# ahmetaa/fast-dnn

Measured on AMD Instinct MI355X. Metric: acoustic frames/sec (whole node), 7x2048->8000 nnet, higher is better.
Workload: dtype int8 (u8 activations x s8 weights -> int32; fp32 layer 0 and soft-max)

## Files before the change

### fast-dnn_amd/api.py

```python
from __future__ import annotations

import ctypes as C
import os
import subprocess
from typing import Optional, Sequence

import numpy as np

_HERE = os.path.dirname(os.path.abspath(__file__))
LIB_PATH = os.environ.get("FDNN_LIB") or os.path.join(_HERE, "lib", "libfast-dnn.so")
CSRC = os.path.join(_HERE, "csrc")

FDNN_OK, FDNN_E_ARG, FDNN_E_IO, FDNN_E_FORMAT, FDNN_E_DEVICE, FDNN_E_NOMEM, FDNN_E_STATE = 0, -1, -2, -3, -4, -5, -6


class FdnnError(RuntimeError):
    def __init__(self, code: int, msg: str):
        super().__init__(f"fdnn error {code}: {msg}")
        self.code = code


def build(verbose: bool = False) -> str:
    jobs = str(max(1, min(8, os.cpu_count() or 1)))
    subprocess.check_call(["make", "-C", CSRC, "-j", jobs, "all"] + ([] if verbose else ["-s"]))
# ... 15 lines not shown
    "fdnn_model_load_on": (C.c_int, [C.c_char_p, C.c_float, C.c_int, C.POINTER(C.c_void_p)]),
    "fdnn_model_free": (None, [C.c_void_p]),
    "fdnn_model_input_dim": (C.c_int, [C.c_void_p]),
    "fdnn_model_output_dim": (C.c_int, [C.c_void_p]),
    "fdnn_model_hidden_dim": (C.c_int, [C.c_void_p]),
    "fdnn_model_layer_count": (C.c_int, [C.c_void_p]),
    "fdnn_model_layer_dim": (C.c_int, [C.c_void_p, C.c_int]),
    "fdnn_model_device": (C.c_int, [C.c_void_p]),
    "fdnn_model_set_l0_fma": (C.c_int, [C.c_void_p, C.c_int]),
    "fdnn_debug_set_l0_kernel": (C.c_int, [C.c_void_p, C.c_int]),
    "fdnn_debug_set_chain": (C.c_int, [C.c_int, C.c_int]),
    "fdnn_model_chain_faults": (C.c_int, [C.c_void_p, C.POINTER(C.c_ulonglong)]),
    "fdnn_debug_set_pp": (C.c_int, [C.c_int, C.c_int]),
    "fdnn_debug_set_ppo": (C.c_int, [C.c_int]),
    "fdnn_debug_launch_name_count": (C.c_int, []),
    "fdnn_debug_launch_name": (C.c_char_p, [C.c_int, C.POINTER(C.c_int)]),
    "fdnn_debug_launch_record": (C.c_int, [C.c_int]),
    "fdnn_debug_launch_reset": (C.c_int, []),
    "fdnn_debug_launch_counts": (C.c_int, [C.POINTER(C.c_ulonglong), C.c_int]),
    "fdnn_debug_raise_fuse_fault": (C.c_int, [C.c_void_p, C.c_int]),
    "fdnn_device_shared": (C.c_int, [C.c_int]),
    "fdnn_debug_set_fuse": (C.c_int, [C.c_int]),
    "fdnn_debug_set_l0_list_cap": (C.c_int, [C.c_void_p, C.c_int]),
    "fdnn_debug_chain_clocks": (C.c_int, [C.c_void_p, C.POINTER(C.c_longlong), C.c_int]),
    "fdnn_calculate": (C.c_int, [C.c_void_p, _c_f32p, C.c_int, C.c_int, C.c_int, _c_f32p]),
    "fdnn_calculate_device": (C.c_int, [C.c_void_p, C.c_void_p, C.c_int, C.c_void_p, C.c_void_p]),
    "fdnn_calculate_lazy": (C.c_int, [C.c_void_p, _c_f32p, C.c_int, C.c_int, _c_i8p, _c_f32p]),
    "fdnn_calculate_lazy_bits": (C.c_int, [C.c_void_p, _c_f32p, C.c_int, C.c_int, C.POINTER(C.c_uint64), _c_f32p]),
    "fdnn_calculate_lazy_bits_device": (C.c_int, [C.c_void_p, C.c_void_p, C.c_int, C.c_void_p, C.c_void_p, C.c_void_p]),
    "fdnn_ctx_create": (C.c_int, [C.c_void_p, C.c_int, C.c_int, C.POINTER(C.c_void_p)]),
    "fdnn_ctx_free": (None, [C.c_void_p]),
    "fdnn_ctx_frame_count": (C.c_int, [C.c_void_p]),
    "fdnn_ctx_output_dim": (C.c_int, [C.c_void_p]),
    "fdnn_ctx_forward_hidden": (C.c_int, [C.c_void_p, _c_f32p]),
    "fdnn_ctx_forward_hidden_device": (C.c_int, [C.c_void_p, C.c_void_p, C.c_void_p]),
    "fdnn_ctx_lazy_output": (C.c_int, [C.c_void_p, C.c_int, _c_i8p, _c_f32p]),
    "fdnn_ctx_lazy_output_batch": (C.c_int, [C.c_void_p, C.c_int, C.c_int, _c_i8p, _c_f32p]),
    "fdnn_ctx_lazy_output_batch_device": (C.c_int, [C.c_void_p, C.c_int, C.c_int, C.c_void_p, C.c_void_p, C.c_void_p]),
    "fdnn_ctx_output": (C.c_int, [C.c_void_p, _c_f32p]),
    "fdnn_ctx_output_device": (C.c_int, [C.c_void_p, C.c_void_p, C.c_void_p]),
    "fdnn_ctx_read_hidden": (C.c_int, [C.c_void_p, _c_u8p]),
    "fdnn_server_create": (C.c_int, [C.c_void_p, C.c_int, C.c_int, C.POINTER(C.c_void_p)]),
    "fdnn_server_free": (None, [C.c_void_p]),
    "fdnn_server_set_linger_us": (C.c_int, [C.c_void_p, C.c_int]),
    "fdnn_server_submit_device": (C.c_int, [C.c_void_p, C.c_void_p, C.c_int, C.c_void_p, C.c_void_p, C.POINTER(C.c_uint64)]),
    "fdnn_server_submit": (C.c_int, [C.c_void_p, _c_f32p, C.c_int, _c_i8p, _c_f32p, C.POINTER(C.c_uint64)]),
# ... 119 lines not shown
def device_shared(device: int = 0) -> bool:
    r = int(lib().fdnn_device_shared(int(device)))
    if r < 0:
        _check(r)
    return r == 1


def set_fuse(mode: int) -> None:
    _check(lib().fdnn_debug_set_fuse(int(mode)))


def set_chain(mode: int, min_frames: int = 0) -> None:
    _check(lib().fdnn_debug_set_chain(int(mode), int(min_frames)))


def set_pp(mode: int, min_frames: int = 0) -> None:
    _check(lib().fdnn_debug_set_pp(int(mode), int(min_frames)))


def set_ppo(mode: int) -> None:
    _check(lib().fdnn_debug_set_ppo(int(mode)))


LAUNCH_ABLATION, LAUNCH_LOAD_TIME = 1, 2


def launch_names() -> dict:
    L = lib()
    out = {}
    for i in range(L.fdnn_debug_launch_name_count()):
        flags = C.c_int(0)
        name = L.fdnn_debug_launch_name(i, C.byref(flags)).decode()
        out[name] = flags.value
    return out


def launch_record(on: bool = True) -> None:
    _check(lib().fdnn_debug_launch_record(1 if on else 0))


def launch_reset() -> None:
    _check(lib().fdnn_debug_launch_reset())


def launch_counts(nonzero: bool = True) -> dict:
    L = lib()
# ... 601 lines not shown
```

### fast-dnn_amd/csrc/fdnn_debug.cpp

```cpp
#include <hip/hip_runtime.h>

#include <algorithm>
#include <atomic>
#include <cstring>
#include <mutex>
#include <string>
#include <vector>

#include "fdnn_internal.hpp"

using namespace fdnn;

struct fdnn_host_model {
  fdnn::HostModel hm;
};

namespace fdnn {
const LaunchNameInfo kLaunchNames[kLaunchNameCount] = {
#define FDNN_X(id, name, flags) {name, flags},
    FDNN_LAUNCH_NAMES(FDNN_X)
#undef FDNN_X
#define FDNN_G(out, shape, branch, name, abl) {name, abl},
        FDNN_GEMM_LAUNCH_NAMES(FDNN_G)
#undef FDNN_G
// ... 32 lines not shown
int fdnn_debug_lazy_expand(float *out, const float *comp, int count, int O, int stride, const uint64_t *bits, int mode) {
  if (!out || !comp || !bits || count < 0 || O <= 0 || stride <= 0 || stride > O + 1 || mode < 0 || mode > 2) return fail(FDNN_E_ARG, "bad argument");
  lazy_expand_force_scalar(mode == 1);
  if (mode == 2) {
    if (stride > O) return fail(FDNN_E_ARG, "the in-place form needs stride <= O");
    std::memmove(out + size_t(count) * size_t(O) - size_t(count) * size_t(stride), comp, sizeof(float) * size_t(count) * size_t(stride));
    fdnn::lazy_expand_rows(out, count, size_t(O), size_t(stride), bits);
  } else {
    fdnn::lazy_expand_rows_from(out, comp, count, size_t(O), size_t(stride), bits);
  }
  lazy_expand_force_scalar(false);
  return FDNN_OK;
}

int fdnn_debug_set_l0_list_cap(fdnn_model *m, int cap) {
  if (!m || cap < 0) return fail(FDNN_E_ARG, "bad argument");
  std::lock_guard<std::mutex> lk(m->mu);
  for (fdnn_ctx *c : m->pool) destroy_ctx(c);
  m->pool.clear();
  m->l0_list_cap = cap;
  return FDNN_OK;
}

int fdnn_debug_set_pp(int mode, int min_frames) {
  if (mode < -1 || mode > 1) return fail(FDNN_E_ARG, "pp mode must be -1, 0 or 1");
  fdnn::qpp_set_mode(mode, min_frames);
  return FDNN_OK;
}

int fdnn_debug_raise_fuse_fault(fdnn_model *m, int value) {
  if (!m) return fail(FDNN_E_ARG, "null model");
  if (!m->h_fuse_fault) return fail(FDNN_E_STATE, "this model has no fault word");
  __atomic_store_n(m->h_fuse_fault, value ? 1ull : 0ull, __ATOMIC_RELAXED);
  if (!value) m->fuse_fault_said = false;
  return FDNN_OK;
}

int fdnn_debug_set_ppo(int mode) {
  if (mode < -1 || mode > 1) return fail(FDNN_E_ARG, "ppo mode must be -1, 0 or 1");
  fdnn::qppo_set_mode(mode);
  return FDNN_OK;
}

int fdnn_debug_launch_name_count(void) { return fdnn::kLaunchNameCount; }

const char *fdnn_debug_launch_name(int index, int *flags) {
// ... 352 lines not shown
```

### fast-dnn_amd/csrc/fdnn_kernels.hpp

```cpp
#pragma once
#include <hip/hip_runtime.h>

#include <cstdint>
#include <vector>

#include "fdnn_note.hpp"

#ifdef FDNN_ABLATION
#include <cstdlib>
#define FDNN_TUNE_ENV(name) std::getenv(name)
#else
#define FDNN_TUNE_ENV(name) static_cast<const char *>(nullptr)
#if (defined(FDNN_GEMM_DEBUG) && FDNN_GEMM_DEBUG) || (defined(FDNN_L0S_DEBUG) && FDNN_L0S_DEBUG) || (defined(FDNN_L0_DEBUG) && FDNN_L0_DEBUG) || \
    (defined(FDNN_CHAIN_CLK) && FDNN_CHAIN_CLK) || defined(FDNN_L0S_CLK) || defined(FDNN_GEMM_PAD)
#error "ablation / clock builds need -DFDNN_ABLATION (tools/build_variant.sh)"
#endif
#endif

namespace fdnn {

constexpr int kMaxFrameTile = 320;
constexpr int kPartialNodes = 64;

struct L0Params {
// ... 15 lines not shown
  float *park;
  int j_pad, jc;
  int n_ld, h_ld;
  const float *wnorm;
  uint32_t *scr_count;
  uint16_t *scr_list;
  unsigned long long *scr_stats;
  int8_t *xd;
  float *xstat;
  const int8_t *wd;
  const float *wstat;
  uint2 *glist;
  uint32_t *glist_count;
  int glist_cap;
  const uint32_t *luthalf;
  float *dbg_t;
  float *dbg_dd;
};
constexpr int kL0ScreenCap = 4096;
void launch_l0(const L0Params &p, hipStream_t s);
bool l0_split_ok(int D, int H);
size_t l0_split_plane_bytes(int D, int rows_ld);
void launch_l0_split(const L0Params &p, hipStream_t s);
void l0_split_build_weights(const float *w, const float *wnorm, const uint8_t *lut2, int H, int D, int h_ld, std::vector<int8_t> *planes,
                            std::vector<float> *stat, std::vector<uint32_t> *half);
int l0_chunk_rows(int D);
int l0_chain_node_tile();
void launch_l0_weight_image(const float *w, float *wt, int H, int D, int j_pad, int h_ld, hipStream_t s);

int qgemm_frame_tile(int rows_pad, int n);
int qgemm_node_tile(int rows_pad, int n, bool output);
int qgemm_debug_flags();

struct QGemmParams {
  const int8_t *w;
  const int8_t *a;
  const float *bias;
  const int32_t *wsum;
  const int32_t *fix_grp;
  const void *fix_ent;
  const uint8_t *lut;
  const uint8_t *lut2;
  int rows, rows_pad, K, n, n_pad;
  int ldw, lda;
  int frame_tile;
  int small;
// ... 91 lines not shown
```

### fast-dnn_amd/csrc/fdnn_l0s.hip

```cpp
#include <atomic>
#include <cmath>
#include <cstdlib>
#include <limits>
#include <type_traits>
#include <vector>

#include "fdnn_device.hpp"
#include "fdnn_kernels.hpp"

namespace fdnn {

namespace {

#ifndef FDNN_L0S_DEBUG
#define FDNN_L0S_DEBUG 0
#endif
constexpr float kU = 5.9604645e-8f;
constexpr int kSplitW = 32;

[[maybe_unused]] __device__ __forceinline__ bool split_tile_of_block(int node_tiles, int frame_tiles, int &bx, int &by) {
  const int b = blockIdx.x, xcd = b & 7, slot = b >> 3;
  bx = slot % node_tiles;
  by = xcd + 8 * (slot / node_tiles);
  return by < frame_tiles;
}

constexpr int kDigFrames = 8;
__global__ __launch_bounds__(256) void l0_digits_kernel(L0Params p, int KC, int J, int JP) {
  extern __shared__ __attribute__((aligned(16))) float dig_smem[];
  const int D = p.D, ld = D + 1;
  float *xs = dig_smem;
  float *cf_s = dig_smem + kDigFrames * ld;
  const int tid = threadIdx.x, f0 = blockIdx.x * kDigFrames;
  if (blockIdx.x == 0 && tid < 2) p.glist_count[tid] = 0u;
  const int quads = D >> 2;
  {
    float4 raw[4], sh[4], sc[4];
    int rowq[4];
#pragma unroll
    for (int it = 0; it < 4; ++it) {
      const int i = tid + it * 256;
      const int row = i / quads, q = i - row * quads, f = f0 + row;
      const bool in = i < kDigFrames * quads;
      rowq[it] = in ? row * ld + 4 * q : -1;
      raw[it] = make_float4(0.f, 0.f, 0.f, 0.f);
      sh[it] = raw[it];
      sc[it] = raw[it];
      if (in && f < p.n) {
// ... 75 lines not shown
      d1[e4] = w1; d2[e4] = w2; d3[e4] = w3;
    }
    const int f = f0 + row;
    if (f >= p.n_ld) continue;
    const size_t blocks = static_cast<size_t>(p.n_ld >> 5);
#pragma unroll
    for (int pl = 0; pl < 3; ++pl) {
      const uint32_t *d = pl == 0 ? d1 : pl == 1 ? d2 : d3;
      char *base = reinterpret_cast<char *>(p.xd) + ((static_cast<size_t>(kc) * 3 + pl) * blocks + (f >> 5)) * 1024 + hh * 512 + (f & 31) * 16;
      *reinterpret_cast<uint4 *>(base) = make_uint4(d[0], d[1], d[2], d[3]);
    }
  }
}

constexpr int kSTF = 128, kSStages = 3;
template <int WN>
struct SplitCfg {
  static constexpr int TN = 64 * WN, NW = 4 * WN, THREADS = 64 * NW;
  static constexpr int PIECES = 12 + 6 * WN;
  static constexpr int STAGE = PIECES * 1024;
  static constexpr int RING = STAGE * kSStages;
  static constexpr int HALF_OFF = RING;
  static constexpr int STAT_OFF = RING + 11 * 1024;
  static constexpr int LDS = STAT_OFF + 3 * 1024;
  static constexpr int TS = TN + 16;
  static constexpr int PPW = (PIECES + NW - 1) / NW;
  static_assert(kSTF * TS + 16 + 2 * kL0ScreenCap <= RING, "epilogue tile and flag list must fit in the dead ring");
};
static_assert(4 * kLut2Size <= 11 * 1024, "half-step table area");

template <int WN, bool DBG = false>
__global__ __launch_bounds__(256 * WN, 3 - WN) void l0_split_kernel(L0Params p, int KC, int CPC) {
#if defined(__HIP_DEVICE_COMPILE__)
  using Cfg = SplitCfg<WN>;
  constexpr int kSTN = Cfg::TN, kSStage = Cfg::STAGE, kSTS = Cfg::TS, kSHalfOff = Cfg::HALF_OFF, kSStatOff = Cfg::STAT_OFF, NW = Cfg::NW;
  extern __shared__ __attribute__((aligned(16))) char smem[];
  const int tid = threadIdx.x, lane = tid & 63;
  const int wave = __builtin_amdgcn_readfirstlane(tid >> 6);
  const int l32 = lane & 31, h = lane >> 5;
  const int wf = wave & 3, wn = wave >> 2;
  const int node_tiles = p.h_ld / kSTN, frame_tiles = (p.n_rows + kSTF - 1) / kSTF;
  int bx, by;
  if (!split_tile_of_block(node_tiles, frame_tiles, bx, by)) return;
  const int f0 = by * kSTF, n0 = bx * kSTN;
  const int xblocks = p.n_ld >> 5, wblocks = p.h_ld >> 5;
#ifdef FDNN_L0S_CLK
  long long tc[12];
  tc[0] = __builtin_readcyclecounter();
#define L0S_TS(i) tc[i] = __builtin_readcyclecounter()
#else
#define L0S_TS(i)
#endif

  {
    const __amdgpu_buffer_rsrc_t rsrc_half =
        __builtin_amdgcn_make_buffer_rsrc(const_cast<uint32_t *>(p.luthalf), 0, (4 * kLut2Size + 15) & ~15, 0x00020000);
#pragma unroll
    for (int i = 0; i < 14; ++i) {
      if (i % NW != wave) continue;
      if (i < 11) {
        __builtin_amdgcn_raw_ptr_buffer_load_lds(rsrc_half, FDNN_LDS_PTR(smem + kSHalfOff + i * 1024), 16, lane * 16, i * 1024, 0, 0);
      } else {
        const int q = i - 11;
        const __amdgpu_buffer_rsrc_t rsrc_st =
            __builtin_amdgcn_make_buffer_rsrc(const_cast<float *>(p.xstat + static_cast<size_t>(q) * p.n_ld + f0), 0, kSTF * 4, 0x00020000);
        __builtin_amdgcn_raw_ptr_buffer_load_lds(rsrc_st, FDNN_LDS_PTR(smem + kSStatOff + q * 1024), 16, lane * 16, 0, 0, 0);
      }
    }
  }
  const __amdgpu_buffer_rsrc_t rsrc_x =
      __builtin_amdgcn_make_buffer_rsrc(const_cast<int8_t *>(p.xd), 0, static_cast<unsigned>(KC) * 3u * static_cast<unsigned>(xblocks) * 1024u, 0x00020000);
  const __amdgpu_buffer_rsrc_t rsrc_w = __builtin_amdgcn_make_buffer_rsrc(
      const_cast<int8_t *>(p.wd), 0, static_cast<unsigned>(KC) * 3u * static_cast<unsigned>(wblocks) * 1024u, 0x00020000);
  const int voff = lane * 16;
  const int my_pieces = (Cfg::PIECES - wave + NW - 1) / NW;
  auto stage_piece = [&](int kc, int buf, int t) {
    char *base = smem + buf * kSStage;
    const int i = wave + NW * t;
    if (i >= Cfg::PIECES) return;
    if (i < 12) {
      const int pl = i >> 2, q = i & 3;
      __builtin_amdgcn_raw_ptr_buffer_load_lds(rsrc_x, FDNN_LDS_PTR(base + i * 1024), 16, voff, ((kc * 3 + pl) * xblocks + (f0 >> 5) + q) * 1024, 0, 0);
    } else {
      const int j = i - 12, pl = j / (2 * WN), q = j % (2 * WN);
      __builtin_amdgcn_raw_ptr_buffer_load_lds(rsrc_w, FDNN_LDS_PTR(base + i * 1024), 16, voff, ((kc * 3 + pl) * wblocks + (n0 >> 5) + q) * 1024, 0, 0);
    }
  };
  auto stage = [&](int kc, int buf) {
#pragma unroll
    for (int t = 0; t < Cfg::PPW; ++t) stage_piece(kc, buf, t);
  };
  auto wait_stages = [&](int stages) {
    if (stages == 0) {
      asm volatile("s_waitcnt vmcnt(0) lgkmcnt(0)" ::: "memory");
    } else if (Cfg::PIECES % NW == 0) {
      if (stages == 1)
        asm volatile("s_waitcnt vmcnt(%0) lgkmcnt(0)" ::"n"(Cfg::PPW) : "memory");
      else
        asm volatile("s_waitcnt vmcnt(%0) lgkmcnt(0)" ::"n"(2 * Cfg::PPW) : "memory");
    } else if (my_pieces == Cfg::PPW) {
// ... 12 lines not shown
  stage(1, 1);
  stage(2, 2);
  asm volatile("" ::: "memory");

  constexpr int kP0Off = 0x40000000;
  v16i P0[2], P1[2], P2[2];
  uint32_t A[2][16];
#pragma unroll
  for (int s = 0; s < 2; ++s)
#pragma unroll
    for (int r = 0; r < 16; ++r) {
      P0[s][r] = kP0Off; P1[s][r] = 0; P2[s][r] = 0;
      A[s][r] = 0u;
    }
  auto chain_end = [&](int s) {
#pragma unroll
    for (int r = 0; r < 16; ++r) {
      P1[s][r] += P0[s][r] << 8;
      P0[s][r] = kP0Off;
    }
  };
  v4i xa[2][3], wb[2][3][2];
  auto load_plane = [&](int buf, int set, int pl) {
    const char *sb = smem + buf * kSStage;
    xa[set][pl] = *reinterpret_cast<const v4i *>(sb + (pl * 4 + wf) * 1024 + lane * 16);
#pragma unroll
    for (int s = 0; s < 2; ++s) wb[set][pl][s] = *reinterpret_cast<const v4i *>(sb + 12288 + (pl * 2 * WN + wn * 2 + s) * 1024 + lane * 16);
  };
  auto load_frags = [&](int buf, int set) {
#pragma unroll
    for (int pl = 0; pl < 3; ++pl) load_plane(buf, set, pl);
  };
  auto sample_part = [&](int ss, int r0, int r1, bool on) {
    if ((FDNN_L0S_DEBUG & 1) || !on) return;
#pragma unroll
    for (int r = r0; r < r1; ++r) asm volatile("v_sad_u32 %0, %1, 2.0, %0" : "+v"(A[ss][r]) : "v"(P0[ss][r]));
  };
#define FDNN_L0S_FENCE __builtin_amdgcn_sched_barrier(0)
  auto mfma_group = [&](int set, int s, int ss, bool on, auto x0, auto x1, auto x2, auto x3, auto x4) {
    FDNN_L0S_FENCE;
    P0[s] = __builtin_amdgcn_mfma_i32_32x32x32_i8(xa[set][0], wb[set][0][s], P0[s], 0, 0, 0);
    if (FDNN_L0S_DEBUG & 2) {
      sample_part(ss, 0, 16, on);
      x0(); x1(); x2(); x3(); x4();
      return;
    }
    FDNN_L0S_FENCE;
// ... 15 lines not shown
    sample_part(ss, 9, 12, on);
    x3();
    FDNN_L0S_FENCE;
    P2[s] = __builtin_amdgcn_mfma_i32_32x32x32_i8(xa[set][1], wb[set][1][s], P2[s], 0, 0, 0);
    FDNN_L0S_FENCE;
    sample_part(ss, 12, 16, on);
    x4();
    FDNN_L0S_FENCE;
    P2[s] = __builtin_amdgcn_mfma_i32_32x32x32_i8(xa[set][2], wb[set][0][s], P2[s], 0, 0, 0);
    FDNN_L0S_FENCE;
  };
  auto nothing = [] {};

  wait_stages(2);
  __builtin_amdgcn_s_barrier();
  asm volatile("" ::: "memory");
  load_frags(0, 0);
  L0S_TS(1);
  auto chunk = [&](int kc, auto set_c, auto first_c, bool chain_start) {
    constexpr int set = decltype(set_c)::value;
    constexpr bool first = decltype(first_c)::value;
    if (chain_start) chain_end(0);
    mfma_group(set, 0, 1, !first, nothing, nothing, nothing, nothing, nothing);
    const bool more = kc + 1 < KC, refill = kc + 3 < KC && !(FDNN_L0S_DEBUG & 8);
    if (more) {
      wait_stages(kc + 2 < KC ? 1 : 0);
      if (!(FDNN_L0S_DEBUG & 16)) __builtin_amdgcn_s_barrier();
      asm volatile("" ::: "memory");
    }
    if (chain_start) chain_end(1);
    const int nb = (kc + 1) % 3;
    mfma_group(
        set, 1, 0, true, [&] { if (more && !(FDNN_L0S_DEBUG & 32)) load_plane(nb, set ^ 1, 0); if (refill) stage_piece(kc + 3, kc % 3, 0); },
        [&] { if (more && !(FDNN_L0S_DEBUG & 32)) load_plane(nb, set ^ 1, 1); if (refill) stage_piece(kc + 3, kc % 3, 1); },
        [&] { if (more && !(FDNN_L0S_DEBUG & 32)) load_plane(nb, set ^ 1, 2); if (refill) stage_piece(kc + 3, kc % 3, 2); },
        [&] { if (refill && Cfg::PPW > 3) stage_piece(kc + 3, kc % 3, 3); }, [&] { if (refill && Cfg::PPW > 4) stage_piece(kc + 3, kc % 3, 4); });
  };
  using C0 = std::integral_constant<int, 0>;
  using C1 = std::integral_constant<int, 1>;
  chunk(0, C0{}, std::true_type{}, false);
  chunk(1, C1{}, std::false_type{}, false);
  for (int kc = 2, in_chain = 2; kc < KC; kc += 2, in_chain += 2) {
    const bool chain_start = in_chain == CPC;
    if (chain_start) in_chain = 0;
    chunk(kc, C0{}, std::false_type{}, chain_start);
    chunk(kc + 1, C1{}, std::false_type{}, false);
  }
  sample_part(1, 0, 16, true);
  chain_end(0);
  chain_end(1);
  L0S_TS(2);

  __syncthreads();
  const char *half_b = smem + kSHalfOff + 4 * kLut2Half;
  const float *rf_s = reinterpret_cast<const float *>(smem + kSStatOff);
  const float *xn_s = rf_s + 256, *af_s = rf_s + 512;
  uint8_t *tile = reinterpret_cast<uint8_t *>(smem);
  uint32_t *scr_n = reinterpret_cast<uint32_t *>(tile + kSTF * kSTS);
  uint16_t *scr_l = reinterpret_cast<uint16_t *>(tile + kSTF * kSTS + 16);
  if (tid == 0) *scr_n = 0;
  const float fD = static_cast<float>(p.D);
  const float c2 = 1.001f * (0.5f * fD * fD + 2.0f * fD) * kU;
  const float kA = 1.00001f * 256.0f * 1.002f * kU * (kSplitW + 3);
  const float kS = 100.001f * 1.002f * kU * (kSplitW / 2 + 2 + c2);
  float bias100[2], rn100[2], kSw2[2], bn2[2], eb2[2];
  bool node_in[2];
#pragma unroll
  for (int s = 0; s < 2; ++s) {
    const int node = n0 + wn * 64 + s * 32 + l32;
    node_in[s] = node < p.H;
    const float b = node_in[s] ? p.bias[node] : 0.0f;
    bias100[s] = 100.0f * b;
    rn100[s] = 100.0f * (node_in[s] ? p.wstat[node] : 0.0f);
    kSw2[s] = kS * (node_in[s] ? p.wstat[p.h_ld + node] : 0.0f);
    bn2[s] = 1.00001f * (node_in[s] ? p.wstat[2 * p.h_ld + node] : 0.0f);
    eb2[s] = 100.001f * 10.0f * kU * fabsf(b);
  }
  uint32_t valid = 0;
#pragma unroll
  for (int r = 0; r < 16; ++r) {
    const bool row_in = f0 + wf * 32 + 8 * (r >> 2) + 4 * h + (r & 3) < p.n;
    valid |= (row_in && node_in[0] ? 1u : 0u) << r;
    valid |= (row_in && node_in[1] ? 1u : 0u) << (16 + r);
  }
  float tt[2][16], sg[2][16];
  uint32_t ent[2][16];
#pragma unroll
  for (int r = 0; r < 16; ++r) {
    const float rf = rf_s[wf * 32 + 8 * (r >> 2) + 4 * h + (r & 3)];
#pragma unroll
    for (int s = 0; s < 2; ++s) {
      const float v = fmaf(static_cast<float>(P2[s][r]), 0.00390625f, static_cast<float>(P1[s][r]));
      sg[s][r] = rf * rn100[s];
      tt[s][r] = fmaf(v, sg[s][r], bias100[s]);
      const int u = max(-kLut2Half, min(kLut2Half, static_cast<int>(tt[s][r] + tt[s][r])));
      ent[s][r] = *reinterpret_cast<const uint32_t *>(half_b + 4 * u);
    }
  }
  uint32_t scr_mask = 0;
#pragma unroll
  for (int r = 0; r < 16; ++r) {
    const int row = wf * 32 + 8 * (r >> 2) + 4 * h + (r & 3);
    const float xn = xn_s[row], af = af_s[row];
#pragma unroll
    for (int s = 0; s < 2; ++s) {
      const float t = tt[s][r], sig = sg[s][r];
      tile[row * kSTS + wn * 64 + s * 32 + l32] = static_cast<uint8_t>(ent[s][r]);
      if (!(FDNN_L0S_DEBUG & 4)) {
        const float e = __builtin_amdgcn_fractf(t) - 0.5f;
        const float Dd = fmaf(fabsf(t), 12.0f * kU, fmaf(sig, fmaf(kA, static_cast<float>(A[s][r]), af + bn2[s]), fmaf(kSw2[s], xn, eb2[s]))) + 1e-30f;
        const float gate = __builtin_bit_cast(float, ent[s][r] & 0xffff0000u);
        const float m = fmaxf(fmaxf(fabsf(e), gate), fabsf(t) - 641.0f);
        const bool flag = !(m > Dd) | !(fabsf(t) < 1.0e9f);
        scr_mask |= flag ? (1u << (16 * s + r)) : 0u;
        if (DBG && ((valid >> (16 * s + r)) & 1u)) {
          const size_t o = static_cast<size_t>(f0 + row) * p.H + (n0 + wn * 64 + s * 32 + l32);
          p.dbg_t[o] = t;
          p.dbg_dd[o] = Dd;
        }
      }
    }
  }
  scr_mask &= valid;
  L0S_TS(3);
  __syncthreads();
  L0S_TS(4);
  {
    const int mine = __popc(scr_mask);
    int incl = mine;
#pragma unroll
    for (int off = 1; off < 64; off <<= 1) {
      const int v = __shfl_up(incl, off);
      if (lane >= off) incl += v;
    }
    const int wave_total = __shfl(incl, 63);
    if (wave_total) {
      uint32_t base = 0;
      if (lane == 63) base = atomicAdd(scr_n, static_cast<uint32_t>(wave_total));
      base = __shfl(base, 63);
      uint32_t at = base + static_cast<uint32_t>(incl - mine);
      uint32_t m = scr_mask;
      while (m) {
        const int i = __ffs(m) - 1;
        m &= m - 1;
        const int r = i & 15, sb2 = i >> 4;
        const int row = wf * 32 + 8 * (r >> 2) + 4 * h + (r & 3), col = wn * 64 + sb2 * 32 + l32;
        if (at < static_cast<uint32_t>(kL0ScreenCap)) scr_l[at] = static_cast<uint16_t>(row * kSTN + col);
        ++at;
      }
    }
  }
#pragma unroll
  for (int q = 0; q < kSTF * (kSTN / 16) / Cfg::THREADS; ++q) {
    const int item = tid + q * Cfg::THREADS, row = item / (kSTN / 16), c16 = (item % (kSTN / 16)) * 16;
    const int f = f0 + row;
    if (f < p.n_rows && n0 + c16 < p.H)
      *reinterpret_cast<uint4 *>(p.act_out + static_cast<size_t>(f) * p.act_ld + n0 + c16) = *reinterpret_cast<const uint4 *>(tile + row * kSTS + c16);
  }
  __syncthreads();
  {
    const uint32_t cnt = *scr_n;
    uint32_t *gbase_s = scr_n + 1;
    if (tid == 0) {
      uint32_t gb = 0xffffffffu, fill_from = 0xffffffffu;
      if (cnt != 0 && cnt <= static_cast<uint32_t>(kL0ScreenCap)) {
        gb = atomicAdd(p.glist_count, cnt);
        if (gb + cnt > static_cast<uint32_t>(p.glist_cap)) {
          fill_from = gb;
          gb = 0xffffffffu;
        }
      }
      if (cnt != 0 && gb == 0xffffffffu) {
        p.scr_count[by * (p.h_ld / 128) + (n0 >> 7)] = cnt;
        atomicAdd(p.glist_count + 1, 1u);
      }
      *gbase_s = gb;
      gbase_s[1] = fill_from;
    }
    __syncthreads();
    const uint32_t gb = *gbase_s, fill_from = gbase_s[1];
    if (fill_from < static_cast<uint32_t>(p.glist_cap))
      for (uint32_t i = fill_from + tid; i < static_cast<uint32_t>(p.glist_cap); i += Cfg::THREADS) p.glist[i] = make_uint2(0xffffffffu, 0xffffffffu);
    if (gb != 0xffffffffu)
      for (uint32_t i = tid; i < cnt; i += Cfg::THREADS) {
        const uint32_t e = scr_l[i];
        p.glist[gb + i] = make_uint2(static_cast<uint32_t>(f0) + e / kSTN, static_cast<uint32_t>(n0) + e % kSTN);
      }
  }
#ifdef FDNN_L0S_CLK
  L0S_TS(5);
  if (p.scr_stats && lane == 0 && wave == 0 && (blockIdx.x == 0 || blockIdx.x == gridDim.x / 2 + 3)) {
    unsigned long long *o = p.scr_stats + 4 + (blockIdx.x == 0 ? 0 : 12);
    for (int i = 0; i < 6; ++i) o[i] = static_cast<unsigned long long>(tc[i] - tc[0]);
  }
#endif
#endif
}

}

bool l0_split_ok(int D, int H) { return D >= 64 && D <= 496 && (D & 3) == 0 && (H & 15) == 0; }
int l0_split_chain_pad(int D) { return (D / 4 + 63) / 64 * 64; }
int l0_split_chunks(int D) { return 4 * l0_split_chain_pad(D) / 32; }
size_t l0_split_plane_bytes(int D, int rows_ld) { return static_cast<size_t>(l0_split_chunks(D)) * 3 * static_cast<size_t>(rows_ld / 32) * 1024; }
size_t l0_split_half_bytes() { return (4 * size_t(kLut2Size) + 15) & ~size_t(15); }

void l0_split_build_weights(const float *w, const float *wnorm, const uint8_t *lut2, int H, int D, int h_ld, std::vector<int8_t> *planes,
                            std::vector<float> *stat, std::vector<uint32_t> *half) {
  const int J = D / 4, JP = l0_split_chain_pad(D);
  planes->assign(l0_split_plane_bytes(D, h_ld), 0);
  stat->assign(static_cast<size_t>(3) * h_ld, 0.0f);
  half->assign(l0_split_half_bytes() / 4, 0);
  auto at = [&](int u) { return lut2[std::max(-kLut2Half, std::min(kLut2Half, u)) + kLut2Half]; };
  for (int u = -kLut2Half; u <= kLut2Half; ++u) {
    const int mag = u < 0 ? -u : u;
    bool same;
// ... 22 lines not shown
      const int c = pp / JP, j = pp - c * JP, k = 4 * j + c;
      if (j >= J) continue;
      const long W = degenerate ? 0 : std::lrint(static_cast<double>(row[k]) * static_cast<double>(cn));
      n1W += static_cast<double>(W < 0 ? -W : W);
      const int x3 = static_cast<int8_t>(W & 0xff), r = static_cast<int>((W - x3) >> 8), x2 = static_cast<int8_t>(r & 0xff), x1 = (r - x2) >> 8;
      n1W2 += std::abs(x2);
      n1W3 += std::abs(x3);
      const int digit[3] = {x1, x2, x3};
      const int kc = pp >> 5, hh = (pp >> 4) & 1, e = pp & 15;
      for (int pl = 0; pl < 3; ++pl)
        (*planes)[((static_cast<size_t>(kc) * 3 + pl) * blocks + (n >> 5)) * 1024 + hh * 512 + (n & 31) * 16 + e] = static_cast<int8_t>(digit[pl]);
    }
    const double b_n = (u * (kSplitW + 3) * m * 0.502 * n1W / 65536.0 + std::ldexp(0.5 * n1W, -32) + std::ldexp(128.0 * (n1W2 + n1W3), -24) +
                        std::ldexp(128.0 * n1W3, -32)) * 1.002;
    auto up = [](double v) {
      float f = static_cast<float>(v);
      if (static_cast<double>(f) < v) f = std::nextafter(f, std::numeric_limits<float>::infinity());
      return f;
    };
    (*stat)[n] = 256.0f / cn;
    (*stat)[static_cast<size_t>(h_ld) + n] = wnorm[n];
    (*stat)[static_cast<size_t>(2) * h_ld + n] = degenerate ? std::numeric_limits<float>::infinity() : up(256.0 * b_n);
  }
}

void launch_l0_split(const L0Params &p, hipStream_t s) {
  const int KC = l0_split_chunks(p.D), J = p.D / 4, JP = l0_split_chain_pad(p.D);
  static std::atomic<unsigned long long> attr_set{0};
  int dev = 0;
  (void)hipGetDevice(&dev);
  const unsigned long long dev_bit = 1ull << (dev & 63);
  const int dig_lds = (kDigFrames * (p.D + 1) + kDigFrames) * 4;
  static const int wn_forced = [] {
    const char *e = FDNN_TUNE_ENV("FDNN_L0S_WN");
    return e ? std::atoi(e) : 0;
  }();
  const int tiles128 = ((p.n_rows + kSTF - 1) / kSTF) * (p.h_ld / 128);
  const int wn_cfg = wn_forced == 1 || wn_forced == 2 ? wn_forced : (tiles128 <= 128 ? 1 : 2);
  if (!(attr_set.load(std::memory_order_acquire) & dev_bit)) {
    (void)hipFuncSetAttribute(reinterpret_cast<const void *>(l0_split_kernel<1>), hipFuncAttributeMaxDynamicSharedMemorySize, SplitCfg<1>::LDS);
    (void)hipFuncSetAttribute(reinterpret_cast<const void *>(l0_split_kernel<2>), hipFuncAttributeMaxDynamicSharedMemorySize, SplitCfg<2>::LDS);
    attr_set.fetch_or(dev_bit, std::memory_order_release);
  }
  const int frame_tiles = (p.n_rows + kSTF - 1) / kSTF;
  const int dig_rows = frame_tiles * kSTF;
  note_launch(kLn_l0_digits);
  hipLaunchKernelGGL(l0_digits_kernel, dim3(dig_rows / kDigFrames), dim3(256), dig_lds, s, p, KC, J, JP);
  if (p.dbg_t != nullptr && p.dbg_dd != nullptr) {
    (void)hipFuncSetAttribute(reinterpret_cast<const void *>(l0_split_kernel<2, true>), hipFuncAttributeMaxDynamicSharedMemorySize, SplitCfg<2>::LDS);
    note_launch(kLn_l0_split_n128_probe);
    hipLaunchKernelGGL((l0_split_kernel<2, true>), dim3(static_cast<unsigned>(p.h_ld / 128) * ((frame_tiles + 7) / 8) * 8), dim3(512), SplitCfg<2>::LDS, s, p, KC, JP / 32);
    return;
  }
  note_launch(wn_cfg == 2 ? kLn_l0_split_n128 : kLn_l0_split_n64);
  if (wn_cfg == 2)
    hipLaunchKernelGGL(l0_split_kernel<2>, dim3(static_cast<unsigned>(p.h_ld / 128) * ((frame_tiles + 7) / 8) * 8), dim3(512), SplitCfg<2>::LDS, s, p, KC, JP / 32);
  else
    hipLaunchKernelGGL(l0_split_kernel<1>, dim3(static_cast<unsigned>(p.h_ld / 64) * ((frame_tiles + 7) / 8) * 8), dim3(256), SplitCfg<1>::LDS, s, p, KC, JP / 32);
}

}
```

### include/fdnn.h

```cpp
#ifndef FDNN_H
#define FDNN_H

#include <stddef.h>
#include <stdint.h>

#ifdef __cplusplus
extern "C" {
#endif

#define FDNN_API __attribute__((visibility("default")))

typedef enum fdnn_status {
  FDNN_OK = 0,
  FDNN_E_ARG = -1,
  FDNN_E_IO = -2,
  FDNN_E_FORMAT = -3,
  FDNN_E_DEVICE = -4,
  FDNN_E_NOMEM = -5,
  FDNN_E_STATE = -6
} fdnn_status;

typedef struct fdnn_model fdnn_model;
typedef struct fdnn_ctx fdnn_ctx;

// ... 80 lines not shown
FDNN_API int fdnn_group_attach(fdnn_group *g);

FDNN_API int fdnn_model_blob_size(const fdnn_model *m, size_t *bytes);
FDNN_API int fdnn_model_export_blob(const fdnn_model *m, void *d_dst, size_t capacity, void *stream);
FDNN_API int fdnn_model_import_blob(const void *d_src, size_t bytes, int device, fdnn_model **out);

FDNN_API int fdnn_debug_forward_taps(fdnn_model *m, const float *x, int n, const int8_t *masks, float *l0_lin,
                                     uint8_t *u8_acts, int32_t *acc_hid, int32_t *acc_out, float *logits, float *probs);

FDNN_API int fdnn_debug_production_acc_out(fdnn_model *m, const float *x, int n, int stride, const int8_t *masks, int32_t *acc,
                                           float *probs);

FDNN_API int fdnn_debug_frame_chunks(int n, int *chunks, int cap);
FDNN_API int fdnn_debug_frame_chunks_for(int n, int chained, int *chunks, int cap);

FDNN_API int fdnn_debug_set_l0_kernel(fdnn_model *m, int kind);

FDNN_API int fdnn_debug_set_fuse(int mode);

FDNN_API int fdnn_debug_lazy_expand(float *out, const float *comp, int count, int O, int stride, const uint64_t *bits, int mode);

FDNN_API int fdnn_debug_set_l0_list_cap(fdnn_model *m, int cap);

FDNN_API int fdnn_debug_set_chain(int mode, int min_frames);

FDNN_API int fdnn_debug_set_pp(int mode, int min_frames);

FDNN_API int fdnn_debug_set_ppo(int mode);

FDNN_API int fdnn_debug_launch_name_count(void);
FDNN_API const char *fdnn_debug_launch_name(int index, int *flags);
FDNN_API int fdnn_debug_launch_record(int on);
FDNN_API int fdnn_debug_launch_reset(void);
FDNN_API int fdnn_debug_launch_counts(unsigned long long *out, int cap);

FDNN_API int fdnn_debug_raise_fuse_fault(fdnn_model *m, int value);

FDNN_API int fdnn_debug_chain_clocks(fdnn_ctx *c, long long *out, int cap_tasks);

FDNN_API int fdnn_debug_layer0(fdnn_model *m, const float *x, int n, uint8_t *u8_out, unsigned long long *recomputed);

FDNN_API int fdnn_debug_layer0_screen(fdnn_model *m, const float *x, int n, uint8_t *u8_out, float *t_out, float *dd_out,
                                      unsigned long long *recomputed);

FDNN_API int fdnn_device_shared(int device);

// ... 31 lines not shown
```

Before: 16.29 million.

## Make layer-0 split kernel persistent with per-tile node stats staged in LDS

Converts the layer-0 split kernel from one block per tile into a persistent grid capped at CU count times occupancy. Each block loops over virtual tile slots and loads the half-LUT into LDS only once. Per-node bias and weight stats are now staged into a new LDS region with buffer-to-LDS loads, and kernel args are read from the kernarg segment. The global-list atomic reservation is moved ahead of the activation store so its latency can overlap. This aims to cut block launch/prologue cost and scattered global loads, at the cost of extra LDS per block, a loop-carried prologue, and possible load imbalance.

```diff
diff --git a/fast-dnn_amd/api.py b/fast-dnn_amd/api.py
--- a/fast-dnn_amd/api.py
+++ b/fast-dnn_amd/api.py
@@ -61,6 +61,7 @@
     "fdnn_device_shared": (C.c_int, [C.c_int]),
     "fdnn_debug_set_fuse": (C.c_int, [C.c_int]),
     "fdnn_debug_set_l0_list_cap": (C.c_int, [C.c_void_p, C.c_int]),
+    "fdnn_debug_set_l0_grid": (C.c_int, [C.c_int]),
     "fdnn_debug_chain_clocks": (C.c_int, [C.c_void_p, C.POINTER(C.c_longlong), C.c_int]),
     "fdnn_calculate": (C.c_int, [C.c_void_p, _c_f32p, C.c_int, C.c_int, C.c_int, _c_f32p]),
     "fdnn_calculate_device": (C.c_int, [C.c_void_p, C.c_void_p, C.c_int, C.c_void_p, C.c_void_p]),
@@ -226,6 +227,10 @@
     _check(lib().fdnn_debug_set_ppo(int(mode)))
 
 
+def set_l0_grid(cap: int) -> None:
+    _check(lib().fdnn_debug_set_l0_grid(int(cap)))
+
+
 LAUNCH_ABLATION, LAUNCH_LOAD_TIME = 1, 2
 
 
diff --git a/fast-dnn_amd/csrc/fdnn_debug.cpp b/fast-dnn_amd/csrc/fdnn_debug.cpp
--- a/fast-dnn_amd/csrc/fdnn_debug.cpp
+++ b/fast-dnn_amd/csrc/fdnn_debug.cpp
@@ -78,6 +78,12 @@
   return FDNN_OK;
 }
 
+int fdnn_debug_set_l0_grid(int cap) {
+  if (cap < 0) return fail(FDNN_E_ARG, "the grid cap must be >= 0");
+  fdnn::l0_split_set_grid_cap(cap);
+  return FDNN_OK;
+}
+
 int fdnn_debug_set_pp(int mode, int min_frames) {
   if (mode < -1 || mode > 1) return fail(FDNN_E_ARG, "pp mode must be -1, 0 or 1");
   fdnn::qpp_set_mode(mode, min_frames);
diff --git a/fast-dnn_amd/csrc/fdnn_kernels.hpp b/fast-dnn_amd/csrc/fdnn_kernels.hpp
--- a/fast-dnn_amd/csrc/fdnn_kernels.hpp
+++ b/fast-dnn_amd/csrc/fdnn_kernels.hpp
@@ -61,6 +61,7 @@
 bool l0_split_ok(int D, int H);
 size_t l0_split_plane_bytes(int D, int rows_ld);
 void launch_l0_split(const L0Params &p, hipStream_t s);
+void l0_split_set_grid_cap(int cap);
 void l0_split_build_weights(const float *w, const float *wnorm, const uint8_t *lut2, int H, int D, int h_ld, std::vector<int8_t> *planes,
                             std::vector<float> *stat, std::vector<uint32_t> *half);
 int l0_chunk_rows(int D);
diff --git a/fast-dnn_amd/csrc/fdnn_l0s.hip b/fast-dnn_amd/csrc/fdnn_l0s.hip
--- a/fast-dnn_amd/csrc/fdnn_l0s.hip
+++ b/fast-dnn_amd/csrc/fdnn_l0s.hip
@@ -1,3 +1,4 @@
+#include <algorithm>
 #include <atomic>
 #include <cmath>
 #include <cstdlib>
@@ -18,12 +19,6 @@
 constexpr float kU = 5.9604645e-8f;
 constexpr int kSplitW = 32;
 
-[[maybe_unused]] __device__ __forceinline__ bool split_tile_of_block(int node_tiles, int frame_tiles, int &bx, int &by) {
-  const int b = blockIdx.x, xcd = b & 7, slot = b >> 3;
-  bx = slot % node_tiles;
-  by = xcd + 8 * (slot / node_tiles);
-  return by < frame_tiles;
-}
 
 constexpr int kDigFrames = 8;
 __global__ __launch_bounds__(256) void l0_digits_kernel(L0Params p, int KC, int J, int JP) {
@@ -145,7 +140,8 @@
   static constexpr int RING = STAGE * kSStages;
   static constexpr int HALF_OFF = RING;
   static constexpr int STAT_OFF = RING + 11 * 1024;
-  static constexpr int LDS = STAT_OFF + 3 * 1024;
+  static constexpr int NODE_OFF = STAT_OFF + 3 * 1024;
+  static constexpr int LDS = NODE_OFF + 4 * 1024;
   static constexpr int TS = TN + 16;
   static constexpr int PPW = (PIECES + NW - 1) / NW;
   static_assert(kSTF * TS + 16 + 2 * kL0ScreenCap <= RING, "epilogue tile and flag list must fit in the dead ring");
@@ -156,49 +152,68 @@
 __global__ __launch_bounds__(256 * WN, 3 - WN) void l0_split_kernel(L0Params p, int KC, int CPC) {
 #if defined(__HIP_DEVICE_COMPILE__)
   using Cfg = SplitCfg<WN>;
-  constexpr int kSTN = Cfg::TN, kSStage = Cfg::STAGE, kSTS = Cfg::TS, kSHalfOff = Cfg::HALF_OFF, kSStatOff = Cfg::STAT_OFF, NW = Cfg::NW;
+  constexpr int kSTN = Cfg::TN, kSStage = Cfg::STAGE, kSTS = Cfg::TS, kSHalfOff = Cfg::HALF_OFF, kSStatOff = Cfg::STAT_OFF, kSNodeOff = Cfg::NODE_OFF, NW = Cfg::NW;
   extern __shared__ __attribute__((aligned(16))) char smem[];
-  const int tid = threadIdx.x, lane = tid & 63;
-  const int wave = __builtin_amdgcn_readfirstlane(tid >> 6);
-  const int l32 = lane & 31, h = lane >> 5;
-  const int wf = wave & 3, wn = wave >> 2;
   const int node_tiles = p.h_ld / kSTN, frame_tiles = (p.n_rows + kSTF - 1) / kSTF;
-  int bx, by;
-  if (!split_tile_of_block(node_tiles, frame_tiles, bx, by)) return;
-  const int f0 = by * kSTF, n0 = bx * kSTN;
   const int xblocks = p.n_ld >> 5, wblocks = p.h_ld >> 5;
 #ifdef FDNN_L0S_CLK
-  long long tc[12];
-  tc[0] = __builtin_readcyclecounter();
+  long long tc[6], tc_first[6];
+  int tiles_done = 0;
 #define L0S_TS(i) tc[i] = __builtin_readcyclecounter()
 #else
 #define L0S_TS(i)
 #endif
 
-  {
-    const __amdgpu_buffer_rsrc_t rsrc_half =
-        __builtin_amdgcn_make_buffer_rsrc(const_cast<uint32_t *>(p.luthalf), 0, (4 * kLut2Size + 15) & ~15, 0x00020000);
-#pragma unroll
-    for (int i = 0; i < 14; ++i) {
-      if (i % NW != wave) continue;
-      if (i < 11) {
-        __builtin_amdgcn_raw_ptr_buffer_load_lds(rsrc_half, FDNN_LDS_PTR(smem + kSHalfOff + i * 1024), 16, lane * 16, i * 1024, 0, 0);
-      } else {
-        const int q = i - 11;
-        const __amdgpu_buffer_rsrc_t rsrc_st =
-            __builtin_amdgcn_make_buffer_rsrc(const_cast<float *>(p.xstat + static_cast<size_t>(q) * p.n_ld + f0), 0, kSTF * 4, 0x00020000);
-        __builtin_amdgcn_raw_ptr_buffer_load_lds(rsrc_st, FDNN_LDS_PTR(smem + kSStatOff + q * 1024), 16, lane * 16, 0, 0, 0);
-      }
-    }
-  }
+  const __amdgpu_buffer_rsrc_t rsrc_half =
+      __builtin_amdgcn_make_buffer_rsrc(const_cast<uint32_t *>(p.luthalf), 0, (4 * kLut2Size + 15) & ~15, 0x00020000);
+  bool half_in = false;
   const __amdgpu_buffer_rsrc_t rsrc_x =
       __builtin_amdgcn_make_buffer_rsrc(const_cast<int8_t *>(p.xd), 0, static_cast<unsigned>(KC) * 3u * static_cast<unsigned>(xblocks) * 1024u, 0x00020000);
   const __amdgpu_buffer_rsrc_t rsrc_w = __builtin_amdgcn_make_buffer_rsrc(
       const_cast<int8_t *>(p.wd), 0, static_cast<unsigned>(KC) * 3u * static_cast<unsigned>(wblocks) * 1024u, 0x00020000);
-  const int voff = lane * 16;
+  using KArgs = const __attribute__((address_space(4))) L0Params;
+
+  const int virt = node_tiles * ((frame_tiles + 7) >> 3) * 8;
+  for (int v = blockIdx.x; v < virt; v += gridDim.x) {
+  const int vslot = v >> 3, bx = vslot % node_tiles, by = (v & 7) + 8 * (vslot / node_tiles);
+  if (by >= frame_tiles) continue;
+  const int f0 = by * kSTF, n0 = bx * kSTN;
+  int tid = threadIdx.x;
+  asm volatile("" : "+v"(tid));
+  const int lane = tid & 63, l32 = lane & 31, h = lane >> 5, voff = lane * 16;
+  const int wave = __builtin_amdgcn_readfirstlane(tid >> 6), wf = wave & 3, wn = wave >> 2;
   const int my_pieces = (Cfg::PIECES - wave + NW - 1) / NW;
+  int lds0 = 0, kcn = KC;
+  asm volatile("" : "+s"(lds0), "+s"(kcn));
+  char *const sm = smem + lds0;
+  L0S_TS(0);
+  if (!half_in) {
+    half_in = true;
+#pragma unroll
+    for (int i = 0; i < 11; ++i)
+      if (i % NW == wave) __builtin_amdgcn_raw_ptr_buffer_load_lds(rsrc_half, FDNN_LDS_PTR(sm + kSHalfOff + i * 1024), 16, lane * 16, i * 1024, 0, 0);
+  }
+  {
+    KArgs *kt = (KArgs *)__builtin_amdgcn_kernarg_segment_ptr();
+    asm volatile("" : "+s"(kt));
+    const int nodes_in = max(0, min(kSTN, kt->H - n0));
+#pragma unroll
+    for (int i = 0; i < ((FDNN_L0S_DEBUG & 64) ? 3 : 7); ++i) {
+      if (i % NW != wave) continue;
+      if (i < 3) {
+        const __amdgpu_buffer_rsrc_t rsrc_st =
+            __builtin_amdgcn_make_buffer_rsrc(const_cast<float *>(kt->xstat + static_cast<size_t>(i) * kt->n_ld + f0), 0, kSTF * 4, 0x00020000);
+        __builtin_amdgcn_raw_ptr_buffer_load_lds(rsrc_st, FDNN_LDS_PTR(sm + kSStatOff + i * 1024), 16, lane * 16, 0, 0, 0);
+      } else {
+        const int q = i - 3;
+        const float *src = q == 0 ? kt->bias + n0 : kt->wstat + static_cast<size_t>(q - 1) * kt->h_ld + n0;
+        const __amdgpu_buffer_rsrc_t rsrc_nd = __builtin_amdgcn_make_buffer_rsrc(const_cast<float *>(src), 0, nodes_in * 4, 0x00020000);
+        __builtin_amdgcn_raw_ptr_buffer_load_lds(rsrc_nd, FDNN_LDS_PTR(sm + kSNodeOff + q * 1024), 16, lane * 16, 0, 0, 0);
+      }
+    }
+  }
   auto stage_piece = [&](int kc, int buf, int t) {
-    char *base = smem + buf * kSStage;
+    char *base = sm + buf * kSStage;
     const int i = wave + NW * t;
     if (i >= Cfg::PIECES) return;
     if (i < 12) {
@@ -257,7 +272,7 @@
   };
   v4i xa[2][3], wb[2][3][2];
   auto load_plane = [&](int buf, int set, int pl) {
-    const char *sb = smem + buf * kSStage;
+    const char *sb = sm + buf * kSStage;
     xa[set][pl] = *reinterpret_cast<const v4i *>(sb + (pl * 4 + wf) * 1024 + lane * 16);
 #pragma unroll
     for (int s = 0; s < 2; ++s) wb[set][pl][s] = *reinterpret_cast<const v4i *>(sb + 12288 + (pl * 2 * WN + wn * 2 + s) * 1024 + lane * 16);
@@ -319,9 +334,9 @@
     constexpr bool first = decltype(first_c)::value;
     if (chain_start) chain_end(0);
     mfma_group(set, 0, 1, !first, nothing, nothing, nothing, nothing, nothing);
-    const bool more = kc + 1 < KC, refill = kc + 3 < KC && !(FDNN_L0S_DEBUG & 8);
+    const bool more = kc + 1 < kcn, refill = kc + 3 < kcn && !(FDNN_L0S_DEBUG & 8);
     if (more) {
-      wait_stages(kc + 2 < KC ? 1 : 0);
+      wait_stages(kc + 2 < kcn ? 1 : 0);
       if (!(FDNN_L0S_DEBUG & 16)) __builtin_amdgcn_s_barrier();
       asm volatile("" ::: "memory");
     }
@@ -337,7 +352,7 @@
   using C1 = std::integral_constant<int, 1>;
   chunk(0, C0{}, std::true_type{}, false);
   chunk(1, C1{}, std::false_type{}, false);
-  for (int kc = 2, in_chain = 2; kc < KC; kc += 2, in_chain += 2) {
+  for (int kc = 2, in_chain = 2; kc < kcn; kc += 2, in_chain += 2) {
     const bool chain_start = in_chain == CPC;
     if (chain_start) in_chain = 0;
     chunk(kc, C0{}, std::false_type{}, chain_start);
@@ -349,34 +364,40 @@
   L0S_TS(2);
 
   __syncthreads();
-  const char *half_b = smem + kSHalfOff + 4 * kLut2Half;
-  const float *rf_s = reinterpret_cast<const float *>(smem + kSStatOff);
+  KArgs *ka_ptr = (KArgs *)__builtin_amdgcn_kernarg_segment_ptr();
+  asm volatile("" : "+s"(ka_ptr));
+  KArgs &ka = *ka_ptr;
+  const float fD = static_cast<float>(ka.D);
+  const float c2 = 1.001f * (0.5f * fD * fD + 2.0f * fD) * kU;
+  const float kA = 1.00001f * 256.0f * 1.002f * kU * (kSplitW + 3);
+  const float kS = 100.001f * 1.002f * kU * (kSplitW / 2 + 2 + c2);
+  const char *half_b = sm + kSHalfOff + 4 * kLut2Half;
+  const float *rf_s = reinterpret_cast<const float *>(sm + kSStatOff);
   const float *xn_s = rf_s + 256, *af_s = rf_s + 512;
-  uint8_t *tile = reinterpret_cast<uint8_t *>(smem);
+  uint8_t *tile = reinterpret_cast<uint8_t *>(sm);
   uint32_t *scr_n = reinterpret_cast<uint32_t *>(tile + kSTF * kSTS);
   uint16_t *scr_l = reinterpret_cast<uint16_t *>(tile + kSTF * kSTS + 16);
   if (tid == 0) *scr_n = 0;
-  const float fD = static_cast<float>(p.D);
-  const float c2 = 1.001f * (0.5f * fD * fD + 2.0f * fD) * kU;
-  const float kA = 1.00001f * 256.0f * 1.002f * kU * (kSplitW + 3);
-  const float kS = 100.001f * 1.002f * kU * (kSplitW / 2 + 2 + c2);
+  const float *nd_s = reinterpret_cast<const float *>(sm + kSNodeOff);
   float bias100[2], rn100[2], kSw2[2], bn2[2], eb2[2];
   bool node_in[2];
 #pragma unroll
   for (int s = 0; s < 2; ++s) {
-    const int node = n0 + wn * 64 + s * 32 + l32;
-    node_in[s] = node < p.H;
-    const float b = node_in[s] ? p.bias[node] : 0.0f;
+    const int col = wn * 64 + s * 32 + l32;
+    node_in[s] = n0 + col < ka.H;
+    const int node = n0 + col;
+    const bool glob = (FDNN_L0S_DEBUG & 64) != 0;
+    const float b = !glob ? nd_s[col] : node_in[s] ? ka.bias[node] : 0.0f;
     bias100[s] = 100.0f * b;
-    rn100[s] = 100.0f * (node_in[s] ? p.wstat[node] : 0.0f);
-    kSw2[s] = kS * (node_in[s] ? p.wstat[p.h_ld + node] : 0.0f);
-    bn2[s] = 1.00001f * (node_in[s] ? p.wstat[2 * p.h_ld + node] : 0.0f);
+    rn100[s] = 100.0f * (!glob ? nd_s[256 + col] : node_in[s] ? ka.wstat[node] : 0.0f);
+    kSw2[s] = kS * (!glob ? nd_s[512 + col] : node_in[s] ? ka.wstat[ka.h_ld + node] : 0.0f);
+    bn2[s] = 1.00001f * (!glob ? nd_s[768 + col] : node_in[s] ? ka.wstat[2 * ka.h_ld + node] : 0.0f);
     eb2[s] = 100.001f * 10.0f * kU * fabsf(b);
   }
   uint32_t valid = 0;
 #pragma unroll
   for (int r = 0; r < 16; ++r) {
-    const bool row_in = f0 + wf * 32 + 8 * (r >> 2) + 4 * h + (r & 3) < p.n;
+    const bool row_in = f0 + wf * 32 + 8 * (r >> 2) + 4 * h + (r & 3) < ka.n;
     valid |= (row_in && node_in[0] ? 1u : 0u) << r;
     valid |= (row_in && node_in[1] ? 1u : 0u) << (16 + r);
   }
@@ -411,9 +432,9 @@
         const bool flag = !(m > Dd) | !(fabsf(t) < 1.0e9f);
         scr_mask |= flag ? (1u << (16 * s + r)) : 0u;
         if (DBG && ((valid >> (16 * s + r)) & 1u)) {
-          const size_t o = static_cast<size_t>(f0 + row) * p.H + (n0 + wn * 64 + s * 32 + l32);
-          p.dbg_t[o] = t;
-          p.dbg_dd[o] = Dd;
+          const size_t o = static_cast<size_t>(f0 + row) * ka.H + (n0 + wn * 64 + s * 32 + l32);
+          ka.dbg_t[o] = t;
+          ka.dbg_dd[o] = Dd;
         }
       }
     }
@@ -427,14 +448,14 @@
     int incl = mine;
 #pragma unroll
     for (int off = 1; off < 64; off <<= 1) {
-      const int v = __shfl_up(incl, off);
+      const int v = __builtin_amdgcn_ds_bpermute(4 * max(lane - off, 0), incl);
       if (lane >= off) incl += v;
     }
-    const int wave_total = __shfl(incl, 63);
+    const int wave_total = __builtin_amdgcn_readlane(incl, 63);
     if (wave_total) {
       uint32_t base = 0;
       if (lane == 63) base = atomicAdd(scr_n, static_cast<uint32_t>(wave_total));
-      base = __shfl(base, 63);
+      base = __builtin_amdgcn_readlane(base, 63);
       uint32_t at = base + static_cast<uint32_t>(incl - mine);
       uint32_t m = scr_mask;
       while (m) {
@@ -447,48 +468,59 @@
       }
     }
   }
+  __syncthreads();
+  const uint32_t cnt = *scr_n;
+  uint32_t *gbase_s = scr_n + 1;
+  const bool reserve = tid == 0 && cnt != 0 && cnt <= static_cast<uint32_t>(kL0ScreenCap);
+  uint32_t gb_mine = 0xffffffffu;
+  if (reserve && !(FDNN_L0S_DEBUG & 128)) gb_mine = atomicAdd(ka.glist_count, cnt);
 #pragma unroll
   for (int q = 0; q < kSTF * (kSTN / 16) / Cfg::THREADS; ++q) {
     const int item = tid + q * Cfg::THREADS, row = item / (kSTN / 16), c16 = (item % (kSTN / 16)) * 16;
     const int f = f0 + row;
-    if (f < p.n_rows && n0 + c16 < p.H)
-      *reinterpret_cast<uint4 *>(p.act_out + static_cast<size_t>(f) * p.act_ld + n0 + c16) = *reinterpret_cast<const uint4 *>(tile + row * kSTS + c16);
-  }
-  __syncthreads();
+    if (f < ka.n_rows && n0 + c16 < ka.H)
+      *reinterpret_cast<uint4 *>(ka.act_out + static_cast<size_t>(f) * ka.act_ld + n0 + c16) = *reinterpret_cast<const uint4 *>(tile + row * kSTS + c16);
+  }
+  if (reserve && (FDNN_L0S_DEBUG & 128)) gb_mine = atomicAdd(ka.glist_count, cnt);
   {
-    const uint32_t cnt = *scr_n;
-    uint32_t *gbase_s = scr_n + 1;
     if (tid == 0) {
-      uint32_t gb = 0xffffffffu, fill_from = 0xffffffffu;
-      if (cnt != 0 && cnt <= static_cast<uint32_t>(kL0ScreenCap)) {
-        gb = atomicAdd(p.glist_count, cnt);
-        if (gb + cnt > static_cast<uint32_t>(p.glist_cap)) {
-          fill_from = gb;
-          gb = 0xffffffffu;
-        }
+      uint32_t gb = gb_mine, fill_from = 0xffffffffu;
+      if (reserve && gb + cnt > static_cast<uint32_t>(ka.glist_cap)) {
+        fill_from = gb;
+        gb = 0xffffffffu;
       }
       if (cnt != 0 && gb == 0xffffffffu) {
-        p.scr_count[by * (p.h_ld / 128) + (n0 >> 7)] = cnt;
-        atomicAdd(p.glist_count + 1, 1u);
+        ka.scr_count[by * (ka.h_ld / 128) + (n0 >> 7)] = cnt;
+        atomicAdd(ka.glist_count + 1, 1u);
       }
       *gbase_s = gb;
       gbase_s[1] = fill_from;
     }
     __syncthreads();
     const uint32_t gb = *gbase_s, fill_from = gbase_s[1];
-    if (fill_from < static_cast<uint32_t>(p.glist_cap))
-      for (uint32_t i = fill_from + tid; i < static_cast<uint32_t>(p.glist_cap); i += Cfg::THREADS) p.glist[i] = make_uint2(0xffffffffu, 0xffffffffu);
+    if (fill_from < static_cast<uint32_t>(ka.glist_cap)) {
+      uint32_t none = 0xffffffffu;
+      asm volatile("" : "+v"(none));
+      for (uint32_t i = fill_from + tid; i < static_cast<uint32_t>(ka.glist_cap); i += Cfg::THREADS) ka.glist[i] = make_uint2(none, none);
+    }
     if (gb != 0xffffffffu)
       for (uint32_t i = tid; i < cnt; i += Cfg::THREADS) {
         const uint32_t e = scr_l[i];
-        p.glist[gb + i] = make_uint2(static_cast<uint32_t>(f0) + e / kSTN, static_cast<uint32_t>(n0) + e % kSTN);
-      }
-  }
+        ka.glist[gb + i] = make_uint2(static_cast<uint32_t>(f0) + e / kSTN, static_cast<uint32_t>(n0) + e % kSTN);
+      }
+  }
+  L0S_TS(5);
 #ifdef FDNN_L0S_CLK
-  L0S_TS(5);
-  if (p.scr_stats && lane == 0 && wave == 0 && (blockIdx.x == 0 || blockIdx.x == gridDim.x / 2 + 3)) {
+  if (tiles_done++ == 0)
+    for (int i = 0; i < 6; ++i) tc_first[i] = tc[i];
+#endif
+  __syncthreads();
+  }
+#ifdef FDNN_L0S_CLK
+  if (p.scr_stats && threadIdx.x == 0 && tiles_done && (blockIdx.x == 0 || blockIdx.x == gridDim.x / 2 + 3)) {
     unsigned long long *o = p.scr_stats + 4 + (blockIdx.x == 0 ? 0 : 12);
-    for (int i = 0; i < 6; ++i) o[i] = static_cast<unsigned long long>(tc[i] - tc[0]);
+    for (int i = 0; i < 6; ++i) o[i] = static_cast<unsigned long long>(tc_first[i] - tc_first[0]);
+    for (int i = 0; i < 6; ++i) o[6 + i] = tiles_done > 1 ? static_cast<unsigned long long>(tc[i] - tc[0]) : 0ull;
   }
 #endif
 #endif
@@ -557,6 +589,26 @@
     (*stat)[static_cast<size_t>(h_ld) + n] = wnorm[n];
     (*stat)[static_cast<size_t>(2) * h_ld + n] = degenerate ? std::numeric_limits<float>::infinity() : up(256.0 * b_n);
   }
+}
+
+static std::atomic<int> g_split_grid_cap{0};
+void l0_split_set_grid_cap(int cap) { g_split_grid_cap.store(cap, std::memory_order_relaxed); }
+
+static int split_cu_count(int dev) {
+  static std::atomic<int> cus[64];
+  int n = cus[dev & 63].load(std::memory_order_acquire);
+  if (n == 0) {
+    if (hipDeviceGetAttribute(&n, hipDeviceAttributeMultiprocessorCount, dev) != hipSuccess || n <= 0) n = 256;
+    cus[dev & 63].store(n, std::memory_order_release);
+  }
+  return n;
+}
+
+static unsigned split_grid(int dev, int wn, unsigned slots) {
+  unsigned g = std::min(slots, std::max(8u, static_cast<unsigned>(split_cu_count(dev) * (3 - wn)) & ~7u));
+  const int cap = g_split_grid_cap.load(std::memory_order_relaxed);
+  if (cap > 0) g = std::min(g, static_cast<unsigned>(cap));
+  return g;
 }
 
 void launch_l0_split(const L0Params &p, hipStream_t s) {
@@ -581,17 +633,18 @@
   const int dig_rows = frame_tiles * kSTF;
   note_launch(kLn_l0_digits);
   hipLaunchKernelGGL(l0_digits_kernel, dim3(dig_rows / kDigFrames), dim3(256), dig_lds, s, p, KC, J, JP);
+  const unsigned slots128 = static_cast<unsigned>(p.h_ld / 128) * ((frame_tiles + 7) / 8) * 8;
   if (p.dbg_t != nullptr && p.dbg_dd != nullptr) {
     (void)hipFuncSetAttribute(reinterpret_cast<const void *>(l0_split_kernel<2, true>), hipFuncAttributeMaxDynamicSharedMemorySize, SplitCfg<2>::LDS);
     note_launch(kLn_l0_split_n128_probe);
-    hipLaunchKernelGGL((l0_split_kernel<2, true>), dim3(static_cast<unsigned>(p.h_ld / 128) * ((frame_tiles + 7) / 8) * 8), dim3(512), SplitCfg<2>::LDS, s, p, KC, JP / 32);
+    hipLaunchKernelGGL((l0_split_kernel<2, true>), dim3(split_grid(dev, 2, slots128)), dim3(512), SplitCfg<2>::LDS, s, p, KC, JP / 32);
     return;
   }
   note_launch(wn_cfg == 2 ? kLn_l0_split_n128 : kLn_l0_split_n64);
   if (wn_cfg == 2)
-    hipLaunchKernelGGL(l0_split_kernel<2>, dim3(static_cast<unsigned>(p.h_ld / 128) * ((frame_tiles + 7) / 8) * 8), dim3(512), SplitCfg<2>::LDS, s, p, KC, JP / 32);
+    hipLaunchKernelGGL(l0_split_kernel<2>, dim3(split_grid(dev, 2, slots128)), dim3(512), SplitCfg<2>::LDS, s, p, KC, JP / 32);
   else
-    hipLaunchKernelGGL(l0_split_kernel<1>, dim3(static_cast<unsigned>(p.h_ld / 64) * ((frame_tiles + 7) / 8) * 8), dim3(256), SplitCfg<1>::LDS, s, p, KC, JP / 32);
-}
-
-}
+    hipLaunchKernelGGL(l0_split_kernel<1>, dim3(split_grid(dev, 1, 2 * slots128)), dim3(256), SplitCfg<1>::LDS, s, p, KC, JP / 32);
+}
+
+}
diff --git a/include/fdnn.h b/include/fdnn.h
--- a/include/fdnn.h
+++ b/include/fdnn.h
@@ -126,6 +126,8 @@
 
 FDNN_API int fdnn_debug_set_l0_list_cap(fdnn_model *m, int cap);
 
+FDNN_API int fdnn_debug_set_l0_grid(int cap);
+
 FDNN_API int fdnn_debug_set_chain(int mode, int min_frames);
 
 FDNN_API int fdnn_debug_set_pp(int mode, int min_frames);
```

After: 16.35 million, median of 6. Within noise of the previous version (+0.3%).
